# kjeffery/SimplePath

Measured on AMD Instinct MI355X. Metric: Mrays/sec (+ Msamples/sec) at fixed spp; per-pixel L2 vs CPU ref, higher is better.
Workload: dtype f32

## Files before the change

__graft_entry__.py:

```python
from __future__ import annotations

import os
import subprocess
import sys
import tempfile

ROOT = os.path.dirname(os.path.abspath(__file__))


def build() -> None:
    env = dict(os.environ)
    env.setdefault("PYTORCH_ROCM_ARCH", "gfx950")
    jobs = str(min(16, os.cpu_count() or 4))
    subprocess.run(["make", "-s", "-j", jobs, "-C", os.path.join(ROOT, "simplepath_amd")], check=True, env=env)
    subprocess.run(["make", "-s", "-C", os.path.join(ROOT, "tests", "cpp")], check=True, env=env)
    subprocess.run(["make", "-s", "-C", os.path.join(ROOT, "tests", "cpp"), "-f", "wide_visit.mk"], check=True, env=env)
    subprocess.run(["make", "-s", "-C", os.path.join(ROOT, "oracle")], check=True, env=env)
    if os.path.isdir("/root/reference") and os.path.exists(os.path.join(ROOT, "oracle", "build_ref.sh")):
        subprocess.run(["bash", os.path.join(ROOT, "oracle", "build_ref.sh")], check=True, env=env)
    if ROOT not in sys.path:
        sys.path.insert(0, ROOT)
    import simplepath_amd

    simplepath_amd.lib()


def smoke() -> None:
    if ROOT not in sys.path:
        sys.path.insert(0, ROOT)
    import numpy as np

    import simplepath_amd as sp
    from simplepath_amd import scenes
    from tests import _oracle

    d = tempfile.mkdtemp(prefix="sp_smoke_")
    scene = sp.Scene.from_file(scenes.write_bunny_scene(d))
    scene.set_resolution(64, 40)
    scene.upload(device=0, bvh_mode=1)
    tiles = np.arange(0, sp.TileScheduler(64, 40).get_num_tiles(), 3, dtype=np.int32)
    gpu, st = sp.render_tiles(scene, "direct_lighting", 2, tiles)
    cpu, _ = _oracle.render(scene, sp.string_to_integrator_type("direct_lighting"), 2, tiles, variant="spm")
    if not np.array_equal(gpu.view(np.uint32), cpu.view(np.uint32)):
        bad = int(np.sum(gpu != cpu))
        raise AssertionError(f"smoke: GPU radiance differs from the oracle in {bad} values")
    print(f"smoke ok: {tiles.size} tiles, {st.rays} rays, {st.kernel_ms:.3f} ms, bit-exact vs oracle")


if __name__ == "__main__":
    build()
    if len(sys.argv) > 1 and sys.argv[1] == "smoke":
        smoke()
```

simplepath_amd/csrc/hip/sp_mega.hpp:

```cpp
#pragma once
#include "sp_path.hpp"
#include "sp_launch.hpp"

namespace spd {
inline namespace SPD_LAYOUT_NS {

constexpr int WAVES_PER_BLOCK = 4;

template <int INTEG>
__device__ __forceinline__ rgb integrate(Ctx& c, Ray ray)
{
    if constexpr (INTEG == SP_INTEGRATOR_BRUTE_FORCE) return integrate_bruteforce(c, ray);
    else if constexpr (INTEG == SP_INTEGRATOR_BRUTE_FORCE_ITERATIVE) return integrate_iterative<false>(c, ray);
    else if constexpr (INTEG == SP_INTEGRATOR_BRUTE_FORCE_ITERATIVE_RR) return integrate_iterative<true>(c, ray);
    else if constexpr (INTEG == SP_INTEGRATOR_ITERATIVE_RRNEE) return integrate_rrnee(c, ray);
    else if constexpr (INTEG == SP_INTEGRATOR_WHITTED) return integrate_whitted(c, ray);
    else return integrate_direct(c, ray);
}


__device__ __forceinline__ Ray tail_camera_ray(const Scene& sc, uint32_t px, uint32_t py, uint32_t i, const Rsq& q)
{
    const uint32_t seed2d = ((px << 16u) | py) ^ 0x6184faf4u;
    const float    sx     = rseq_component(seed2d, sc.alpha2_0, i);
// ... 152 lines not shown
        }
    }
    asm volatile("s_waitcnt vmcnt(0)" ::: "memory");
    __builtin_amdgcn_fence(__ATOMIC_RELEASE, "agent");
    asm volatile("s_waitcnt vmcnt(0)" ::: "memory");
    if (lane == 0) __hip_atomic_store(ta.ready + k, 1u, __ATOMIC_RELAXED, __HIP_MEMORY_SCOPE_AGENT);
}

__device__ __forceinline__ void tail_chunk(const Scene& sc, const RenderArgs& args, const Rsq& q, Stack& st, int64_t j,
                                           uint32_t lane, uint32_t dx, uint32_t dy, uint32_t& rays_total,
                                           uint32_t& shadow_total, uint32_t& draws_total)
{
    const TailArgs& ta = *args.tail;
    const int64_t   k  = j / ta.chunks;
    const uint32_t  c  = (uint32_t)(j % ta.chunks);
    if (lane == 0)
        while (__hip_atomic_load(ta.ready + k, __ATOMIC_RELAXED, __HIP_MEMORY_SCOPE_AGENT) == 0u) __builtin_amdgcn_s_sleep(4);
    __builtin_amdgcn_fence(__ATOMIC_ACQUIRE, "agent");
    asm volatile("s_waitcnt vmcnt(0)" ::: "memory");
    const int64_t  slot   = args.order ? args.order[k] : k;
    const int32_t  tile   = args.tile_ids ? args.tile_ids[slot] : (int32_t)slot;
    const uint32_t px     = (uint32_t)((tile % args.tiles_x) * 8) + dx;
    const uint32_t py     = (uint32_t)((tile / args.tiles_x) * 8) + dy;
    const bool     inside = px < (uint32_t)sc.width && py < (uint32_t)sc.height;
    const size_t   p      = (size_t)k * 64 + lane;
    const uint32_t i0     = c * ta.chunk_len;
    const uint32_t i1     = min(args.spp, i0 + ta.chunk_len);
    if (!inside || i0 >= i1) return;
    const uint32_t snap = ta.snap_ctl[(size_t)c * ta.n_px + p];
    Rng            rng;
    rng.base  = ta.gens + (size_t)k * ta.gens_per_px * MT_GEN_WORDS + (size_t)lane * MT_BLK;
    rng.idx   = (int)(snap & 0xffffu);
    rng.cur   = (int)(snap >> 16);
    rng.lin   = 1;
    rng.pre   = 1;
    rng.ready = 1;
    rng.draws = 0;
    rng.pfn   = 0;
    Ctx ctx{ sc, rng, q, st, 0u, 0u };
    for (uint32_t i = i0; i < i1; ++i) {
        rng_prepare(rng);
        const float4   rec  = ta.hits[(size_t)i * ta.n_px + p];
        const uint32_t code = __float_as_uint(rec.y);
        if (code == 0xffffffffu) continue;
        const Ray   ray = tail_camera_ray(sc, px, py, i, q);
        const Hit   h{ rec.x, code, rec.z, rec.w };
        const Isect is  = finish_hit(sc, h, ray, q);
        const rgb   L   = direct_nee(ctx, is, neg(ray.d));
        ta.L[((size_t)i * 3 + 0) * ta.n_px + p] = L.r;
        ta.L[((size_t)i * 3 + 1) * ta.n_px + p] = L.g;
        ta.L[((size_t)i * 3 + 2) * ta.n_px + p] = L.b;
    }
    rays_total += ctx.rays;
    shadow_total += ctx.shadow;
    draws_total += rng.draws;
}


__device__ __forceinline__ void resume_copy_gen(const uint64_t* __restrict__ src, uint64_t* __restrict__ dst)
{
    constexpr int U = 6;
    static_assert(MT_ROWS % U == 0, "whole blocks of rows");
#pragma unroll 1
    for (int r0 = 0; r0 < MT_ROWS; r0 += U) {
        if constexpr (MT_BLK % 2 == 0) {
            ulonglong2 w[U][MT_BLK / 2];
#pragma unroll
            for (int j = 0; j < U; ++j)
#pragma unroll
                for (int b = 0; b < MT_BLK / 2; ++b)
                    w[j][b] = reinterpret_cast<const ulonglong2*>(src + (size_t)(r0 + j) * (64 * MT_BLK))[b];
#pragma unroll
            for (int j = 0; j < U; ++j)
#pragma unroll
                for (int b = 0; b < MT_BLK / 2; ++b)
                    reinterpret_cast<ulonglong2*>(dst + (size_t)(r0 + j) * (64 * MT_BLK))[b] = w[j][b];
        } else {
            uint64_t w[U][MT_BLK];
#pragma unroll
            for (int j = 0; j < U; ++j)
#pragma unroll
                for (int b = 0; b < MT_BLK; ++b) w[j][b] = src[(size_t)(r0 + j) * (64 * MT_BLK) + b];
#pragma unroll
            for (int j = 0; j < U; ++j)
#pragma unroll
                for (int b = 0; b < MT_BLK; ++b) dst[(size_t)(r0 + j) * (64 * MT_BLK) + b] = w[j][b];
        }
    }
}

__device__ __forceinline__ void resume_load(Rng& r, const ResumeArgs& ra, int64_t slot, int lane, rgb& acc)
{
    const size_t p = (size_t)slot * 64 + lane;
    resume_copy_gen(ra.gen + (size_t)slot * MT_GEN_WORDS + (size_t)lane * MT_BLK, mt_buf(r, 0));
    r.cur   = 0;
    r.idx   = (int)ra.pos[p];
    r.ready = 0;
    r.draws = 0;
    r.pfn   = 0;
#if SP_SERVE_RHO
    r.srv_on = 0;
    r.srv_A  = false;
    r.srv_B  = false;
#endif
    const float* s = ra.sum + (size_t)slot * 192 + lane;
    acc            = mkc(s[0], s[64], s[128]);
}

__device__ __forceinline__ void resume_save(Rng& r, const ResumeArgs& ra, int64_t slot, int lane, rgb acc)
{
    const size_t p  = (size_t)slot * 64 + lane;
    const bool   sw = r.idx >= MT_N && r.ready != 0;
    resume_copy_gen(mt_buf(r, sw ? mt_next(r) : r.cur), ra.gen + (size_t)slot * MT_GEN_WORDS + (size_t)lane * MT_BLK);
    ra.pos[p] = sw ? 0u : (uint32_t)r.idx;
    ra.draws[p] += r.draws;
    float* s = ra.sum + (size_t)slot * 192 + lane;
    s[0]     = acc.r;
    s[64]    = acc.g;
    s[128]   = acc.b;
}

__device__ __forceinline__ void noise_push(float& mean, float& m2, rgb L, uint32_t n)
{
    const float y = ((0.2126f * L.r) + (0.7152f * L.g)) + (0.0722f * L.b);
    if (n == 1) {
        mean = y;
        m2   = 0.0f;
    } else {
        const float d = y - mean;
        mean          = mean + d / (float)n;
        m2            = m2 + d * (y - mean);
    }
}

template <int INTEG, bool PROBE, int TAIL = 0, bool RESUME = false, bool ADAPT = false>
__device__ __forceinline__ void render_tiles_body(const Scene& sc, const RenderArgs& args, const ResumeArgs* res = nullptr,
                                                  const AdaptArgs* ad = nullptr)
{
    static_assert(!RESUME || (!PROBE && TAIL == 0), "progressive calls run the plain megakernel form");
    static_assert(!ADAPT || RESUME, "adaptive calls are progressive calls");
    extern __shared__ uint32_t lds[];
    const int tid  = threadIdx.x;
    const int lane = tid & 63;
    const int wave = tid >> 6;
    const int rs_words = rsqrt_words(sc);
    for (int i = tid; i < rs_words; i += 64 * WAVES_PER_BLOCK) lds[i] = sc.rsqrt_entries[i];
    libm_lds_init(tid, 64 * WAVES_PER_BLOCK);
#ifdef SP_WAVE_PROF
    if (lane < 16) wprof_lds[wave * 16 + lane] = 0;
#endif
#ifdef SP_TRAFFIC_DIAG
    if (lane < 32) tdg_lds[wave * 32 + lane] = 0;
#endif
    __syncthreads();
    Rsq   q{ lds };
    Stack st{ lds + rs_words + wave * sc.stack_words * 64, lane, sc.stack_depth };

    const size_t gwave = (size_t)blockIdx.x * WAVES_PER_BLOCK + wave;
    Rng          rng;
    rng.base = args.mt_state + gwave * (2 * (size_t)MT_GEN_WORDS) + (size_t)lane * MT_BLK;

    uint32_t rays_total = 0, shadow_total = 0, samples_total = 0, draws_total = 0;
    if constexpr (PROBE) rng_seed(rng, (uint32_t)(gwave * 64 + lane) ^ 0xb0ae9d99u);
    const uint32_t dx = morton_decode_1((uint32_t)lane);
    const uint32_t dy = morton_decode_1((uint32_t)lane >> 1);
    int64_t        n_active = 0;
    if constexpr (ADAPT) n_active = *ad->n_active;
    while (true) {
        int grabbed = 0;
        if (lane == 0) grabbed = atomicAdd(args.tile_counter, 1);
        const int64_t item = __shfl(grabbed, 0, 64);
        if constexpr (ADAPT) {
            if (item >= n_active) break;
        } else if constexpr (TAIL == 2) {
            {
                const int64_t NC = args.tail_cam;
                if (item < NC) {
                    fused_camera(sc, args, q, st, item, (uint32_t)lane, dx, dy);
                    continue;
                }
                const int64_t it = item - NC;
                const int64_t K = args.tail_prep, C = args.tail_items / max<int64_t>(1, K), P = min(args.tail_front, K);
                if (it >= K + args.tail_items) break;
                int64_t   idx  = it;
                bool      prep = it < P;
                if (!prep) {
                    const int64_t j = it - P, full = K - P;
                    if (j < full * (C + 1)) {
                        const int64_t g = j / (C + 1), r = j % (C + 1);
                        prep            = r == C;
                        idx             = prep ? g + P : g * C + r;
                    } else {
                        idx = full * C + (j - full * (C + 1));
                    }
                }
                if (prep) tail_prep<true>(sc, args, q, st, idx, (uint32_t)lane, dx, dy, rays_total, samples_total);
                else tail_chunk(sc, args, q, st, idx, (uint32_t)lane, dx, dy, rays_total, shadow_total, draws_total);
                continue;
            }
        } else if constexpr (TAIL == 1 || TAIL == 3) {
            if (item >= args.num_tiles + args.tail_items) break;
            if (item < args.tail_prep) {
                tail_prep<false, TAIL == 3>(sc, args, q, st, item, (uint32_t)lane, dx, dy, rays_total, samples_total);
                continue;
            }
            if (item >= args.num_tiles) {
                tail_chunk(sc, args, q, st, item - args.num_tiles, (uint32_t)lane, dx, dy, rays_total, shadow_total,
                           draws_total);
                continue;
            }
        } else if (item * (PROBE ? (int64_t)args.probe_step : 1) >= args.num_tiles) {
            break;
        }
        int64_t slot;
        if constexpr (ADAPT) slot = __builtin_amdgcn_readfirstlane(ad->active[item]);
        else slot = PROBE ? item * args.probe_step : (args.order ? args.order[item] : item);
        const uint64_t t_start = (PROBE || args.tile_diag) ? __builtin_amdgcn_s_memrealtime() : 0;
        const int32_t  tile   = args.tile_ids ? args.tile_ids[slot] : (int32_t)slot;
        const uint32_t px     = (uint32_t)((tile % args.tiles_x) * 8) + dx;
        const uint32_t py     = (uint32_t)((tile / args.tiles_x) * 8) + dy;
        const bool     inside = px < (uint32_t)sc.width && py < (uint32_t)sc.height;
        rgb            acc    = mkc(0, 0, 0);
        uint64_t       prof[4] = { 0, 0, 0, 0 };
        uint32_t       a_n0 = 0, a_more = 0;
        if constexpr (ADAPT) {
            a_n0   = __builtin_amdgcn_readfirstlane(ad->done[slot]);
            a_more = a_n0 < ad->cap ? min(ad->step, ad->cap - a_n0) : 0u;
        }
        if (inside) {
            const uint32_t pix_seed = (px << 16u) | py;
            float nz_mean = 0.0f, nz_m2 = 0.0f;
            if constexpr (ADAPT) {
                if (a_n0 == 0) {
                    rng_seed_twisted(rng, pix_seed ^ 0xb0ae9d99u);
                } else {
                    resume_load(rng, *res, slot, lane, acc);
                    nz_mean = ad->mean[(size_t)slot * 64 + lane];
                    nz_m2   = ad->m2[(size_t)slot * 64 + lane];
                }
            } else if constexpr (RESUME) {
                if (res->n0 == 0) rng_seed_twisted(rng, pix_seed ^ 0xb0ae9d99u);
                else resume_load(rng, *res, slot, lane, acc);
            } else if constexpr (!PROBE) {
                if (SP_SEED_FUSED) rng_seed_twisted(rng, pix_seed ^ 0xb0ae9d99u);
                else rng_seed(rng, pix_seed ^ 0xb0ae9d99u);
            }
            const uint32_t seed2d = pix_seed ^ 0x6184faf4u;
            Ctx c{ sc, rng, q, st, 0u, 0u };
            if (args.deep) {
                c.deep    = args.deep + gwave * 64 + lane;
                c.dstride = args.deep_stride;
            }
            uint32_t i_first = 0, i_end = args.spp;
            if constexpr (ADAPT) {
                i_first = a_n0;
                i_end   = a_n0 + a_more;
            } else if constexpr (RESUME) {
                i_first = res->n0;
                i_end   = res->n0 + args.spp;
            }
            for (uint32_t i = i_first; i < i_end; ++i) {
                rng_prepare(rng);
                const float sx = rseq_component(seed2d, sc.alpha2_0, i);
                const float sy = rseq_component(seed2d, sc.alpha2_1, i);
                const float fx = (float)(int)px + sx;
                const float fy = (float)(int)py + sy;
                Ray ray;
                ray.o = sc.camera.p;
                ray.d = normalize(add(add(scale(fx, sc.camera.vx), scale(fy, sc.camera.vy)), sc.camera.vz), q);
                if constexpr (ADAPT) {
                    rgb L;
                    if constexpr (INTEG == SP_INTEGRATOR_MANDELBROT) L = integrate_mandelbrot(fx, fy, sc.width, sc.height);
                    else SP_WPROF(0, L = integrate<INTEG>(c, ray));
                    acc = cadd(acc, L);
                    noise_push(nz_mean, nz_m2, L, i + 1u);
                } else if constexpr (INTEG == SP_INTEGRATOR_MANDELBROT)
                    acc = cadd(acc, integrate_mandelbrot(fx, fy, sc.width, sc.height));
                else
                    SP_WPROF(0, acc = cadd(acc, integrate<INTEG>(c, ray)));
            }
            if constexpr (RESUME) resume_save(rng, *res, slot, lane, acc);
            if constexpr (ADAPT) {
                ad->mean[(size_t)slot * 64 + lane] = nz_mean;
                ad->m2[(size_t)slot * 64 + lane]   = nz_m2;
            }
            acc = cdivs(acc, (float)i_end);
#ifdef SP_MEGA_PROF
            for (int k = 0; k < 4; ++k) prof[k] = c.prof[k];
#endif
            rays_total += c.rays;
            shadow_total += c.shadow;
            samples_total += ADAPT ? a_more : args.spp;
            draws_total += rng.draws;
        }
        if constexpr (ADAPT)
            if (lane == 0) ad->done[slot] = a_n0 + a_more;
        if constexpr (PROBE) {
            if (lane == 0) args.tile_time[slot] = (float)(__builtin_amdgcn_s_memrealtime() - t_start);
            continue;
        }
        if constexpr (RESUME)
            if (!args.out) continue;
        float* o = args.out + ((size_t)slot * 64 + lane) * 3;
        o[0]     = acc.r;
        o[1]     = acc.g;
        o[2]     = acc.b;
#if !defined(SP_WAVE_PROF) && !defined(SP_TRAFFIC_DIAG)
        if (args.tile_diag) {
            for (int k = 0; k < 4; ++k)
                for (int off = 32; off > 0; off >>= 1) {
                    const uint64_t o = __shfl_xor(prof[k], off, 64);
                    prof[k]          = o > prof[k] ? o : prof[k];
                }
            const uint64_t t_end  = __builtin_amdgcn_s_memrealtime();
            const uint64_t rec[8] = { t_start, t_end, (uint64_t)gwave, (uint64_t)item, prof[0], prof[1], prof[2], prof[3] };
            if (lane < 8) args.tile_diag[(size_t)slot * 8 + lane] = rec[lane];
        }
#endif
    }
#ifdef SP_WAVE_PROF
    if (args.tile_diag && lane < 16) atomicAdd(args.tile_diag + lane, wprof_lds[wave * 16 + lane]);
#endif
#ifdef SP_TRAFFIC_DIAG
    if (args.tile_diag && lane < 32) atomicAdd(args.tile_diag + 16 + lane, tdg_lds[wave * 32 + lane]);
#endif
    unsigned long long v[4] = { rays_total, shadow_total, samples_total, draws_total };
    for (int k = 0; k < 4; ++k) {
        unsigned long long s = v[k];
        for (int off = 32; off > 0; off >>= 1) s += __shfl_down(s, off, 64);
        if (lane == 0 && s) atomicAdd(args.counters + k, s);
    }
}
template <int INTEG, int MINW>
__global__ void __launch_bounds__(64 * WAVES_PER_BLOCK, MINW) sp_render_kernel(Scene sc, RenderArgs args)
{
    render_tiles_body<INTEG, false>(sc, args);
}
template <int INTEG, int MINW>
__global__ void __launch_bounds__(64 * WAVES_PER_BLOCK, MINW) sp_probe_kernel(Scene sc, RenderArgs args)
{
    render_tiles_body<INTEG, true>(sc, args);
}
template <int INTEG, int MINW>
__global__ void __launch_bounds__(64 * WAVES_PER_BLOCK, MINW) sp_resume_kernel(Scene sc, RenderArgs args, ResumeArgs res)
{
    render_tiles_body<INTEG, false, 0, true>(sc, args, &res);
}
template <int INTEG, int MINW>
__global__ void __launch_bounds__(64 * WAVES_PER_BLOCK, MINW) sp_adapt_kernel(Scene sc, RenderArgs args, ResumeArgs res, AdaptArgs ad)
{
    render_tiles_body<INTEG, false, 0, true, true>(sc, args, &res, &ad);
}
template <int MINW, bool REPLAY>
__global__ void __launch_bounds__(64 * WAVES_PER_BLOCK, MINW) sp_tail_kernel(Scene sc, RenderArgs args)
{
    render_tiles_body<SP_INTEGRATOR_DIRECT_LIGHTING, false, REPLAY ? 3 : 1>(sc, args);
}
template <int MINW>
__global__ void __launch_bounds__(64 * WAVES_PER_BLOCK, MINW) sp_fused_kernel(Scene sc, RenderArgs args)
{
    render_tiles_body<SP_INTEGRATOR_DIRECT_LIGHTING, false, 2>(sc, args);
}
}

using KernelFn = void (*)(Scene, RenderArgs);
KernelFn mega_direct(int variant);
KernelFn mega_iterative(int integ);
KernelFn mega_rrnee(int waves);
KernelFn mega_recursive(int integ);
KernelFn mega_mandelbrot();
KernelFn probe_direct(int variant);
KernelFn probe_rrnee(int waves);
KernelFn tail_direct(int variant, bool replay);
KernelFn fused_chunks();
using ResumeFn = void (*)(Scene, RenderArgs, ResumeArgs);
ResumeFn   resume_direct(int variant);
ResumeFn   resume_mandelbrot();
ResumeFn   resume_rrnee(int waves);
ResumeFn   resume_path(int integ);
ResumeFn   select_resume(int integ, int variant);
using AdaptFn = void (*)(Scene, RenderArgs, ResumeArgs, AdaptArgs);
AdaptFn    adapt_direct(int variant);
AdaptFn    adapt_mandelbrot();
AdaptFn    adapt_rrnee(int waves);
AdaptFn    adapt_path(int integ);
AdaptFn    select_adapt(int integ, int variant);

}
```

simplepath_amd/csrc/hip/sp_path.hpp:

```cpp
#pragma once
#include "sp_device.hpp"
#include "../common/sp_wide_visit.h"

namespace spd {
inline namespace SPD_LAYOUT_NS {

using namespace spm;

#ifdef SP_WAVE_PROF
static __shared__ unsigned long long wprof_lds[16 * 16];
__device__ __forceinline__ void wprof_end(int k, uint64_t t0)
{
    const uint64_t dt    = __builtin_amdgcn_s_memtime() - t0;
    const uint64_t m     = __ballot(1);
    const int      first = __ffsll((unsigned long long)m) - 1;
    if ((int)(threadIdx.x & 63) == first) {
        const int w = threadIdx.x >> 6;
        wprof_lds[w * 16 + 2 * k] += dt;
        wprof_lds[w * 16 + 2 * k + 1] += dt * (uint64_t)__popcll(m);
    }
}
#define SP_WPROF(k, stmt)                                                                                              \
    do {                                                                                                               \
        const uint64_t t_wp_ = __builtin_amdgcn_s_memtime();                                                           \
        stmt;                                                                                                          \
        wprof_end(k, t_wp_);                                                                                           \
    } while (0)
#else
#define SP_WPROF(k, stmt) stmt
#endif

#ifdef SP_TRAFFIC_DIAG
enum { TD_NODE, TD_TRI, TD_BIN, TD_HIT, TD_DRAW, TD_TOUCH, TD_SERVED, TD_TWIST, TD_SEED, TD_BOUNCE, TD_N };
static __shared__ unsigned long long tdg_lds[16 * 32];
__device__ __forceinline__ void td_add(int cat, uint64_t lines, uint64_t bytes)
{
    const uint64_t m     = __ballot(1);
    const int      first = __ffsll((unsigned long long)m) - 1;
    if ((int)(threadIdx.x & 63) == first) {
        const int w = threadIdx.x >> 6;
        tdg_lds[w * 32 + 2 * cat] += lines;
        tdg_lds[w * 32 + 2 * cat + 1] += bytes;
    }
}
__device__ __forceinline__ uint32_t td_distinct(uint64_t v, uint64_t todo)
{
    uint32_t cnt = 0;
    while (todo) {
        const int      src = __ffsll((unsigned long long)todo) - 1;
        const uint32_t lo  = (uint32_t)__shfl((int)(uint32_t)v, src, 64);
        const uint32_t hi  = (uint32_t)__shfl((int)(uint32_t)(v >> 32), src, 64);
        todo &= ~__ballot(v == (((uint64_t)hi << 32) | lo));
        ++cnt;
    }
    return cnt;
}
__device__ __forceinline__ void td_lines(int cat, const void* p, int nbytes)
{
    const uint64_t a = (uint64_t)(uintptr_t)p, l0 = a >> 7, l1 = (a + (uint64_t)nbytes - 1) >> 7;
    const uint64_t m = __ballot(1);
    uint32_t cnt = td_distinct(l0, m);
    cnt += td_distinct(l1 != l0 ? l1 : ~0ull, __ballot(l1 != l0));
    td_add(cat, cnt, (uint64_t)__popcll(m) * (uint64_t)nbytes);
}
__device__ __forceinline__ void td_twist(int cat)
{
    const uint64_t m = __ballot(1);
    uint64_t groups = 0;
    for (int g = 0; g < 16; ++g) groups += ((m >> (4 * g)) & 0xfull) ? 1 : 0;
    td_add(cat, groups * 78 * 2, (uint64_t)__popcll(m) * 312 * 8 * 2);
}
#define SP_TD(stmt) stmt
#else
#define SP_TD(stmt)
#endif

struct Rsq {
    const uint32_t* t;
};
__device__ __forceinline__ float rsqrt_ref(float a, const Rsq& q)
{
    const uint4    h  = *reinterpret_cast<const uint4*>(q.t);
    const uint32_t hi = q.t[4];
    RsqrtTable     tb{ q.t + RSQ_HDR, (int32_t)h.x, h.y, h.z, (int32_t)h.w, hi };
    return rsqrt_newton(a, rsqrtss_emulated(a, tb));
}
__device__ __forceinline__ f3 normalize(f3 a, const Rsq& q) { return scale(a, rsqrt_ref(dot(a, a), q)); }

#ifndef SP_SQRT_UNIT
#define SP_SQRT_UNIT 1
#endif
__device__ __forceinline__ float sqrt_unit(float x)
{
#if SP_SQRT_UNIT
    const float s  = __builtin_amdgcn_sqrtf(x);
    const float sd = __uint_as_float(__float_as_uint(s) - 1u);
    const float su = __uint_as_float(__float_as_uint(s) + 1u);
    const float vp = __builtin_fmaf(-sd, s, x);
    const float vs = __builtin_fmaf(-su, s, x);
    float       r  = (vp <= 0.0f) ? sd : s;
    r              = (vs > 0.0f) ? su : r;
    return r;
#else
    return sqrt_f(x);
#endif
}

#ifndef SP_RNG_PF
#define SP_RNG_PF 2
#endif
#ifndef SP_XP_SERVED_FREE
#define SP_XP_SERVED_FREE 0
#endif
constexpr int RNG_PF = SP_RNG_PF;
struct Rng {
    uint64_t* base;
    int       cur;
    int       idx;
    int       ready;
    uint32_t  draws;
    int       lin = 0, pre = 0;
    int       pfn = 0;
#ifdef SP_TRAFFIC_DIAG
    int       td_cat = TD_DRAW;
#endif
    uint64_t  pf[RNG_PF > 0 ? RNG_PF : 1];
#if SP_SERVE_RHO
    int       srv_on  = 0;
    bool      srv_A = false, srv_B = false;
    uint32_t  srv_pos = 0, srv_dc = 0, srv_coat = 0, srv_posA = 0, srv_pwA = 0;
#endif
};

__device__ __forceinline__ uint64_t* mt_buf(Rng& r, int b) { return r.base + (size_t)b * MT_GEN_WORDS; }
__device__ __forceinline__ int       mt_next(const Rng& r) { return r.lin ? r.cur + 1 : r.cur ^ 1; }

#ifndef SP_TWIST_BLOCK
#define SP_TWIST_BLOCK 12
#endif
#ifndef SP_TWIST_SKIP_BLOCK
#define SP_TWIST_SKIP_BLOCK 12
#endif
template <int NW, bool SECOND>
__device__ __forceinline__ void mt_twist_words(const uint64_t* __restrict__ A, uint64_t* __restrict__ B, int k, uint64_t& ak)
{
    if constexpr (NW > 0) {
        uint64_t a1[NW], am[NW];
#pragma unroll
        for (int j = 0; j < NW; ++j) {
            a1[j] = A[mt_off(k + j + 1)];
            am[j] = SECOND ? B[mt_off(k + j - (MT_N - MT_M))] : A[mt_off(k + j + MT_M)];
        }
#pragma unroll
        for (int j = 0; j < NW; ++j) {
            B[mt_off(k + j)] = am[j] ^ mt_mix(ak, a1[j]);
// ... 1795 lines not shown
        rho_accumulate(r, mf_sample_geom(m, p, wo, u2, u1, q), m.microfacet_r, grey);
    }
    if (grey) r.g = r.b = r.r;
    return cdivs(r, (float)16u);
}

#if SP_SERVE_RHO
#ifndef SP_MERGE_QUERIES
#define SP_MERGE_QUERIES 1
#endif
enum : int {
    MQ_O = 0,
    MQ_D3 = 192,
    MQ_T3 = 384,
    MQ_D1 = 448,
    MQ_T1 = 640,
    MQ_BEST = 704,
    MQ_ANY = 832,
    MQ_TB = 896,
    MQ_Q = 960,
    MQ_CNT = 992,
    MQ_WORDS = 996,
    SRV_W = 0, SRV_REQ = 512, SRV_WORDS = 576,
    SRV_WAVE_WORDS = (SP_MERGE_QUERIES && MQ_WORDS > SRV_WORDS) ? MQ_WORDS : SRV_WORDS
};
static_assert(SRV_WAVE_WORDS % 4 == 0 && MQ_BEST % 2 == 0, "u64 LDS atomics need 8-byte alignment");
struct MqLayout {
    enum : int { O = MQ_O, D3 = MQ_D3, T3 = MQ_T3, D1 = MQ_D1, T1 = MQ_T1, BEST = MQ_BEST, AMAX = MQ_BEST, ANY = MQ_ANY,
                 TB = MQ_TB, Q = MQ_Q, CNT = MQ_CNT };
};
#ifndef SP_MQ_SHADOW
#define SP_MQ_SHADOW 1
#endif
static __shared__ __attribute__((aligned(16))) uint32_t srv_lds[4][SRV_WAVE_WORDS];
__device__ __forceinline__ float*   srv_w_at(int wave, int k, int j) { return reinterpret_cast<float*>(&srv_lds[wave][SRV_W + (k * 2 + j) * 64]); }
__device__ __forceinline__ uint8_t* srv_req_of(int wave) { return reinterpret_cast<uint8_t*>(&srv_lds[wave][SRV_REQ]); }
#endif

template <bool PAIR = (SP_RNG_PAIR != 0), bool ALIGN = (SP_RHO_ALIGNED != 0), bool TOUCH = (SP_RHO_TOUCH != 0)>
__device__ __forceinline__ void glossy_weights(const Material& m, f3 wo, Rng& rng, const Rsq& q, float w[2])
{
#if SP_SERVE_RHO
    if (rng.srv_on == 1) {
        const uint32_t d = rng.draws - rng.srv_pos;
        int            k = -1;
        if (rng.srv_A && rng.draws == rng.srv_posA) k = 3;
        else if (rng.srv_B) k = (d == 0u) ? 0 : (d == rng.srv_dc) ? 1 : (d == 2u * rng.srv_dc + rng.srv_coat) ? 2 : -1;
        if (k >= 0) {
            const int lane = threadIdx.x & 63, wave = threadIdx.x >> 6;
            w[0]           = srv_w_at(wave, k, 0)[lane];
            w[1]           = srv_w_at(wave, k, 1)[lane];
            rng_skip_reserved(rng, (int)rng.srv_dc);
            return;
        }
    }
#endif
    rgb r0;
    SP_WPROF(1, r0 = (mf_rho16<PAIR, ALIGN, TOUCH>(m, wo, rng, q)));
    const rgb r1 = cscale(m.lambert_albedo, k_pi);
    float     sum = 0.0f;
    w[0] = luminance(r0);
    sum += w[0];
    w[1] = luminance(r1);
    sum += w[1];
    w[0] = w[0] / sum;
    w[1] = w[1] / sum;
}
__device__ __forceinline__ float lambert_only_weight(const Material& m)
{
    const rgb r   = cscale(m.lambert_albedo, k_pi);
    float     sum = 0.0f;
    float     w   = luminance(r);
    sum += w;
    return w / sum;
}
__device__ __forceinline__ float balance(float p, float inner) { return (inner == 0.0f) ? 0.0f : p / inner; }

__device__ __forceinline__ MSample lambert_sample(const Material& m, Rng& rng)
{
    MSample r;
    const P2 u = next2D(rng);
    r.dir      = sample_uniform_hemisphere(u);
    r.color    = m.lambert_albedo;
    r.pdf      = k_uniform_hemisphere_pdf;
    r.props    = PROP_DIFFUSE | PROP_REFLECTIVE;
    return r;
}

__device__ __forceinline__ MSample onesample_sample_w(const Material& m, f3 wo, const float w[2], Rng& rng, const Rsq& q)
{
    const float u   = next1D(rng);
    float       cdf = 0.0f;
    int         sel = 1;
    for (int i = 0; i < 2; ++i) {
        if (w[i] + cdf > u) { sel = i; break; }
        cdf += w[i];
    }
    MSample res = (sel == 0) ? mf_sample(m, wo, rng, q) : lambert_sample(m, rng);
    if (res.pdf == 0.0f || cblack(res.color)) {
        MSample z;
        z.color = mkc(0, 0, 0); z.dir = mk(0, 0, 0); z.pdf = 0.0f; z.props = 0;
        return z;
    }
    const f3 wi = res.dir;
    rgb      values[2];
    float    pdfs[2];
    for (int i = 0; i < 2; ++i) {
        if (i == sel) {
            values[i] = res.color;
            pdfs[i]   = res.pdf * w[i];
        } else if (i == 0) {
            values[i] = mf_eval(m, wo, wi, q);
            pdfs[i]   = mf_pdf(m, wo, wi, q) * w[i];
        } else {
            values[i] = m.lambert_albedo;
            pdfs[i]   = k_uniform_hemisphere_pdf * w[i];
        }
    }
    const float inner = (0.0f + pdfs[0]) + pdfs[1];
    rgb         col   = mkc(0, 0, 0);
    float       pdf   = 0.0f;
    for (int i = 0; i < 2; ++i) {
        if (pdfs[i] > 0.0f) {
            const float mw = balance(pdfs[i], inner);
            col            = cadd(col, cscale(values[i], mw));
            pdf += pdfs[i];
        }
    }
    MSample out;
    out.color = col;
    out.dir   = wi;
    out.pdf   = pdf;
    out.props = res.props;
    return out;
}
__device__ __forceinline__ MSample onesample_sample(const Material& m, f3 wo, Rng& rng, const Rsq& q)
{
    if (m.kind == SP_MAT_LAMBERTIAN) return lambert_sample(m, rng);
    float w[2];
    glossy_weights(m, wo, rng, q, w);
    return onesample_sample_w(m, wo, w, rng, q);
}

__device__ __forceinline__ rgb onesample_eval_w(const Material& m, f3 wo, f3 wi, const float w[2], const Rsq& q)
{
    const float p0    = mf_pdf(m, wo, wi, q) * w[0];
    const float p1    = k_uniform_hemisphere_pdf * w[1];
    const float inner = (0.0f + p0) + p1;
    rgb         r     = mkc(0, 0, 0);
    if (p0 > 0.0f) r = cadd(r, cscale(mf_eval(m, wo, wi, q), balance(p0, inner)));
    if (p1 > 0.0f) r = cadd(r, cscale(m.lambert_albedo, balance(p1, inner)));
    return r;
}
__device__ __forceinline__ rgb onesample_eval(const Material& m, f3 wo, f3 wi, Rng& rng, const Rsq& q)
{
    if (m.kind == SP_MAT_LAMBERTIAN) {
        const float w     = lambert_only_weight(m);
        const float p     = k_uniform_hemisphere_pdf * w;
        const float inner = 0.0f + p;
        rgb         r     = mkc(0, 0, 0);
        if (p > 0.0f) r = cadd(r, cscale(m.lambert_albedo, balance(p, inner)));
        return r;
    }
    float w[2];
    glossy_weights(m, wo, rng, q, w);
    return onesample_eval_w(m, wo, wi, w, q);
}

__device__ __forceinline__ float onesample_pdf_w(const Material& m, f3 wo, f3 wi, const float w[2], const Rsq& q)
{
    float p = 0.0f;
    p += w[0] * mf_pdf(m, wo, wi, q);
    p += w[1] * k_uniform_hemisphere_pdf;
    return p;
}
__device__ __forceinline__ float onesample_pdf(const Material& m, f3 wo, f3 wi, Rng& rng, const Rsq& q)
{
    if (m.kind == SP_MAT_LAMBERTIAN) {
        const float w = lambert_only_weight(m);
        float       p = 0.0f;
        p += w * k_uniform_hemisphere_pdf;
        return p;
    }
    float w[2];
    glossy_weights(m, wo, rng, q, w);
    return onesample_pdf_w(m, wo, wi, w, q);
}

__device__ __forceinline__ bool material_has_rho(const Scene& sc, int mid)
{
    const Material& m = sc.materials[mid];
    const int       k = (m.kind == SP_MAT_CLEARCOAT) ? sc.materials[m.base].kind : m.kind;
    return k == SP_MAT_GLOSSY;
}

__device__ __forceinline__ MSample material_sample_local(const Scene& sc, int mid, f3 wo, Rng& rng, const Rsq& q)
{
    const Material& m    = sc.materials[mid];
    const bool      coat = m.kind == SP_MAT_CLEARCOAT;
    float           f    = 0.0f;
    if (coat) {
        f             = fresnel_dielectric(wo.y, 1.0f, m.coat_ior);
        const float u = next1D(rng);
        if (u < f) {
            MSample s;
            s.dir   = mk(-wo.x, wo.y, -wo.z);
            s.color = cdivs(cscale(m.coat_color, f), abs_f(s.dir.y));
            s.pdf   = f;
            s.props = PROP_SPECULAR | PROP_REFLECTIVE;
            return s;
        }
    }
    const MSample b = onesample_sample(sc.materials[coat ? m.base : mid], wo, rng, q);
    if (!coat || b.pdf == 0.0f) return b;
    MSample s;
    s.pdf   = (1.0f - f) * b.pdf;
    s.color = cmul(csub(mkc(1, 1, 1), cscale(m.coat_color, f)), b.color);
    s.dir   = b.dir;
    s.props = b.props;
    return s;
}
__device__ __forceinline__ rgb material_eval_local(const Scene& sc, int mid, f3 wo, f3 wi, Rng& rng, const Rsq& q)
{
    const Material& m    = sc.materials[mid];
    const bool      coat = m.kind == SP_MAT_CLEARCOAT;
    const rgb       r    = onesample_eval(sc.materials[coat ? m.base : mid], wo, wi, rng, q);
    if (!coat) return r;
    const float f = fresnel_dielectric(wo.y, 1.0f, m.coat_ior);
    return cscale(r, 1.0f - f);
}
__device__ __forceinline__ float material_pdf_local(const Scene& sc, int mid, f3 wo, f3 wi, Rng& rng, const Rsq& q)
{
    const Material& m    = sc.materials[mid];
    const bool      coat = m.kind == SP_MAT_CLEARCOAT;
    const float     p    = onesample_pdf(sc.materials[coat ? m.base : mid], wo, wi, rng, q);
    if (!coat) return p;
    const float f = fresnel_dielectric(wo.y, 1.0f, m.coat_ior);
    return (1.0f - f) * p;
}

__device__ __forceinline__ MSample material_sample(const Scene& sc, int mid, f3 wo_w, f3 n, Rng& rng, const Rsq& q)
{
    const Onb o = onb_from_v(n, q);
    MSample   r = material_sample_local(sc, mid, to_onb(o, wo_w), rng, q);
    if (r.pdf == 0.0f || cblack(r.color)) return r;
    r.dir = to_world(o, r.dir);
    return r;
}
__device__ __forceinline__ rgb material_eval(const Scene& sc, int mid, f3 wo, f3 wi, f3 n, Rng& rng, const Rsq& q)
{
    const Onb o = onb_from_v(n, q);
    return material_eval_local(sc, mid, to_onb(o, wo), to_onb(o, wi), rng, q);
}
__device__ __forceinline__ float material_pdf(const Scene& sc, int mid, f3 wo, f3 wi, f3 n, Rng& rng, const Rsq& q)
{
    const Onb o = onb_from_v(n, q);
    return material_pdf_local(sc, mid, to_onb(o, wo), to_onb(o, wi), rng, q);
}

struct LSample {
    rgb   L;
    float pdf;
    Ray   ray;
    float tmin, tmax;
};

__device__ __forceinline__ float sphere_pdf(const Light& l, f3 observer_world)
{
    const f3    obs = xfm_point(l.w2o, observer_world);
    const float sqr = dot(obs, obs);
    if (sqr <= 1.0f) return k_uniform_sphere_pdf;
    constexpr float sin2_1_5_deg = 0.00068523f;
    const float     sin2_max     = 1.0f / sqr;
    const float     cos_max      = sqrt_unit(std_max(0.0f, 1.0f - sin2_max));
    const float     omc          = (sin2_max < sin2_1_5_deg) ? sin2_max / 2.0f : 1.0f - cos_max;
    return 1.0f / (2.0f * k_pi * omc);
}

__device__ __forceinline__ LSample light_sample(const Scene& sc, const Light& l, f3 obs, f3 obs_n, P2 u, const Rsq& q)
{
    LSample s;
    f3      wi;
    float   pdf, max_dist;
    s.L = l.radiance;
    if (l.kind == SP_LIGHT_SPHERE) {
        const f3 lo = xfm_point(l.w2o, obs);
        f3       local;
        if (dot(lo, lo) <= 1.0f) {
            local = sample_uniform_sphere(u);
        } else {
            const f3  smp = sample_cosine_hemisphere(u);
            const Onb o   = onb_from_v(lo, q);
            local         = to_world(o, smp);
        }
        const f3 sp_w = xfm_point(l.o2w, local);
        const f3 sn_w = xfm_vector(l.nrm, local);
        const f3 to_sample = sub(sp_w, obs);
        wi                 = normalize(to_sample, q);
        pdf                = sphere_pdf(l, obs);
        max_dist           = length(to_sample) - ray_offset(sn_w, neg(wi));
    } else if (l.kind == SP_LIGHT_IMAGE_ENVIRONMENT) {
        const EnvSample es = env_sample(sc.envs[l.image], u);
        wi                 = es.wi;
        pdf                = es.pdf;
        s.L                = es.L;
        max_dist           = k_infinite;
    } else {
        wi       = sample_uniform_sphere(u);
        pdf      = k_uniform_sphere_pdf;
        max_dist = k_infinite;
    }
    s.pdf   = pdf;
    s.tmin  = ray_offset(obs_n, wi);
    s.tmax  = max_dist;
    s.ray.o = obs;
    s.ray.d = wi;
    return s;
}
__device__ __forceinline__ float light_pdf(const Scene& sc, const Light& l, f3 obs, f3 wi)
{
    if (l.kind == SP_LIGHT_SPHERE) return sphere_pdf(l, obs);
    if (l.kind == SP_LIGHT_IMAGE_ENVIRONMENT) return env_pdf(sc.envs[l.image], wi);
    return k_uniform_sphere_pdf;
}

#ifndef SP_OCC_CACHE
#define SP_OCC_CACHE 0
#endif
struct Ctx {
    const Scene& sc;
    Rng&         rng;
    const Rsq&   q;
    Stack        st;
    uint32_t     rays, shadow;
    uint32_t     occ_slot = 0xffffffffu;
    float*       deep    = nullptr;
    size_t       dstride = 0;
#ifdef SP_MEGA_PROF
    uint64_t prof[4] = { 0, 0, 0, 0 };
#endif
};
#ifdef SP_MEGA_PROF
#define SP_PROF(k, stmt)                                                                                               \
    do {                                                                                                               \
        const uint64_t t_prof_ = __builtin_amdgcn_s_memtime();                                                         \
        stmt;                                                                                                          \
        c.prof[k] += __builtin_amdgcn_s_memtime() - t_prof_;                                                           \
    } while (0)
#else
#define SP_PROF(k, stmt) stmt
#endif

__device__ __forceinline__ bool occluded(Ctx& c, const Ray& r, float tmin, float tmax)
{
    ++c.shadow;
    ++c.rays;
    bool hit;
    SP_WPROF(3, hit = scene_any(c.sc, r, tmin, tmax, c.st, SP_OCC_CACHE ? &c.occ_slot : nullptr));
    return hit;
}

struct Query {
    LightHit lh;
    bool     geom;
    Isect    is;
};
__device__ __forceinline__ Query trace(Ctx& c, const Ray& ray, float tmin, float tmax)
{
    Query qr;
    ++c.rays;
    Hit h;
    SP_WPROF(2, {
        qr.lh = scene_intersect_lights(c.sc, ray, tmin, tmax, c.st);
        if (qr.lh.hit) tmax = qr.lh.t;
        h = scene_intersect(c.sc, ray, tmin, tmax, c.st);
    });
    qr.geom     = (h.code != 0xffffffffu);
    if (qr.geom) qr.is = finish_hit(c.sc, h, ray, c.q);
    return qr;
}

__device__ __forceinline__ rgb direct_nee(Ctx& c, const Isect& is, f3 wo)
{
    rgb L = mkc(0, 0, 0);
    for (int li = 0; li < c.sc.n_lights; ++li) {
        const Light l = uload_light(c.sc.lights + li);
        LSample     ls;
        SP_PROF(1, ls = light_sample(c.sc, l, is.p, is.n, next2D(c.rng), c.q));
        if (ls.pdf == 0.0f || cblack(ls.L)) continue;
        const f3 wi = ls.ray.d;
        rgb      f;
        SP_PROF(2, f = material_eval(c.sc, is.material, wo, wi, is.n, c.rng, c.q));
        bool vis = false;
        if (!cblack(f)) SP_PROF(3, vis = !occluded(c, ls.ray, ls.tmin, ls.tmax));
        if (vis) L = cadd(L, cdivs(cscale(cmul(f, ls.L), abs_f(dot(wi, is.n))), ls.pdf));
    }
    return L;
}

__device__ __forceinline__ uint32_t sample_draws(const Scene& sc, const Isect& is, f3 wo, const Rsq& q)
{
    const Material& m    = sc.materials[is.material];
    const int       base = (m.kind == SP_MAT_CLEARCOAT) ? sc.materials[m.base].kind : m.kind;
    bool            rho  = false;
    if (base != SP_MAT_LAMBERTIAN) {
        const Onb o = onb_from_v(is.n, q);
        rho         = to_onb(o, wo).y != 0.0f;
    }
    uint32_t n = 0;
    for (int li = 0; li < sc.n_lights; ++li) {
        const Light lt  = uload_light(sc.lights + li);
        const float pdf = (lt.kind == SP_LIGHT_SPHERE) ? sphere_pdf(lt, is.p) : k_uniform_sphere_pdf;
        n += 2;
        if (rho && !(pdf == 0.0f || cblack(lt.radiance))) n += 32;
    }
    return n;
}

__device__ __forceinline__ rgb integrate_direct(Ctx& c, Ray ray)
{
    rgb L = mkc(0, 0, 0);
    if (0 >= c.sc.max_depth) return L;
    Query qr;
    SP_PROF(0, qr = trace(c, ray, k_ray_epsilon, k_infinite));
    if (qr.geom) {
        L = direct_nee(c, qr.is, neg(ray.d));
    } else if (qr.lh.hit) {
        L = cadd(L, cmul(mkc(1, 1, 1), light_hit_L(c.sc, qr.lh, ray.d, c.q)));
    }
    return L;
}

template <bool RR>
__device__ __forceinline__ rgb integrate_iterative(Ctx& c, Ray ray)
{
    rgb   throughput = mkc(1, 1, 1);
    rgb   L          = mkc(0, 0, 0);
    float tmin = k_ray_epsilon, tmax = k_infinite;
    constexpr float rr_cut = 0.1f;
    for (int depth = 0; depth < c.sc.max_depth; ++depth) {
        rng_prepare(c.rng);
        const Query qr = trace(c, ray, tmin, tmax);
        if (qr.geom) {
            const f3      wo = neg(ray.d);
            const f3      n  = qr.is.n;
            const MSample s  = material_sample(c.sc, qr.is.material, wo, n, c.rng, c.q);
            if (s.pdf == 0.0f || cblack(s.color)) break;
            const f3    wi     = s.dir;
            const float cosine = abs_f(dot(wi, n));
            throughput         = cmul(throughput, cdivs(cscale(s.color, cosine), s.pdf));
            if (RR && depth >= c.sc.rr_depth) {
                const float lum = luminance(throughput);
                if (lum < rr_cut) {
                    const float qv = std_max(0.05f, lum / rr_cut);
                    if (next1D(c.rng) < qv) throughput = cdivs(throughput, qv);
                    else break;
                }
            }
            ray.o = ray_at(ray, qr.is.t);
            ray.d = wi;
            tmin  = ray_offset(cosine);
            tmax  = k_infinite;
        } else if (qr.lh.hit) {
            L = cadd(L, cmul(throughput, light_hit_L(c.sc, qr.lh, ray.d, c.q)));
            break;
        } else {
            break;
        }
    }
    return L;
}

constexpr int MAX_RECURSION = 32;
__device__ __forceinline__ rgb integrate_bruteforce(Ctx& c, Ray ray)
{
    float cosv[MAX_RECURSION];
    rgb   colv[MAX_RECURSION];
    float pdfv[MAX_RECURSION];
    int   depth = 0;
    rgb   Lend  = mkc(0, 0, 0);
    const bool deep = c.deep != nullptr;
    const int  maxd = deep ? c.sc.max_depth : (c.sc.max_depth < MAX_RECURSION ? c.sc.max_depth : MAX_RECURSION);
    auto put = [&](int k, float cs, rgb col, float pdf) {
        if (!deep) { cosv[k] = cs; colv[k] = col; pdfv[k] = pdf; return; }
        float* d = c.deep + (size_t)k * 5 * c.dstride;
        d[0] = cs; d[c.dstride] = col.r; d[2 * c.dstride] = col.g; d[3 * c.dstride] = col.b; d[4 * c.dstride] = pdf;
    };
    while (true) {
        if (depth >= maxd) { Lend = mkc(0, 0, 0); break; }
        rng_prepare(c.rng);
        const Query qr = trace(c, ray, k_ray_epsilon, k_infinite);
        if (qr.geom) {
            const f3      wo = neg(ray.d);
            const f3      n  = qr.is.n;
            const MSample s  = material_sample(c.sc, qr.is.material, wo, n, c.rng, c.q);
            if (s.pdf == 0.0f || cblack(s.color)) { Lend = mkc(0, 0, 0); break; }
            put(depth, dot(s.dir, n), s.color, s.pdf);
            ray.o       = ray_at(ray, qr.is.t);
            ray.d       = s.dir;
            ++depth;
        } else if (qr.lh.hit) {
            Lend = light_hit_L(c.sc, qr.lh, ray.d, c.q);
            break;
        } else {
            Lend = mkc(0, 0, 0);
            break;
        }
    }
    for (int k = depth - 1; k >= 0; --k) {
        float cs, pdf;
        rgb   col;
        if (!deep) { cs = cosv[k]; col = colv[k]; pdf = pdfv[k]; }
        else {
            const float* d = c.deep + (size_t)k * 5 * c.dstride;
            cs = d[0]; col = mkc(d[c.dstride], d[2 * c.dstride], d[3 * c.dstride]); pdf = d[4 * c.dstride];
        }
        Lend = cdivs(cmul(cscale(Lend, cs), col), pdf);
    }
    return Lend;
}

__device__ __forceinline__ rgb integrate_whitted(Ctx& c, Ray ray)
{
    rgb        Lv[MAX_RECURSION + 1];
    int        depth = 0;
    const bool deep  = c.deep != nullptr;
    const int  maxd  = deep ? c.sc.max_depth : (c.sc.max_depth < MAX_RECURSION ? c.sc.max_depth : MAX_RECURSION);
    auto put = [&](int k, rgb L) {
        if (!deep) { Lv[k] = L; return; }
        float* d = c.deep + (size_t)k * 3 * c.dstride;
        d[0] = L.r; d[c.dstride] = L.g; d[2 * c.dstride] = L.b;
    };
    auto get = [&](int k) {
        if (!deep) return Lv[k];
        const float* d = c.deep + (size_t)k * 3 * c.dstride;
        return mkc(d[0], d[c.dstride], d[2 * c.dstride]);
    };
    while (true) {
        rgb L = mkc(0, 0, 0);
        if (depth >= maxd) { put(depth, L); break; }
        rng_prepare(c.rng);
        const Query qr   = trace(c, ray, k_ray_epsilon, k_infinite);
        bool        more = false;
        if (qr.geom) {
            const f3 wo = neg(ray.d);
            L           = direct_nee(c, qr.is, wo);
            if (depth < c.sc.max_depth) {
                const MSample s = material_sample(c.sc, qr.is.material, wo, qr.is.n, c.rng, c.q);
// ... 501 lines not shown
```

Before: 4023.

## Reorder NEE to trace shadow ray first and skip glossy weights when occluded

Direct-light NEE now casts the shadow ray before evaluating glossy material weights. When the ray is occluded and interval bounds prove whether the contribution is black, the costly glossy_weights RNG-driven estimate is skipped and its 32 RNG draws are reserved and skipped to keep the sequence aligned. This removes per-light BRDF estimation on occluded samples. The trade-off is shadow rays are now traced even when the BRDF would have been black, and the ray/shadow counters are adjusted to match the old accounting. A debug check mode is added behind a macro.

```diff
diff --git a/__graft_entry__.py b/__graft_entry__.py
--- a/__graft_entry__.py
+++ b/__graft_entry__.py
@@ -15,6 +15,7 @@
     subprocess.run(["make", "-s", "-j", jobs, "-C", os.path.join(ROOT, "simplepath_amd")], check=True, env=env)
     subprocess.run(["make", "-s", "-C", os.path.join(ROOT, "tests", "cpp")], check=True, env=env)
     subprocess.run(["make", "-s", "-C", os.path.join(ROOT, "tests", "cpp"), "-f", "wide_visit.mk"], check=True, env=env)
+    subprocess.run(["make", "-s", "-j", "3", "-C", os.path.join(ROOT, "tests", "cpp"), "-f", "nee_order.mk"], check=True, env=env)
     subprocess.run(["make", "-s", "-C", os.path.join(ROOT, "oracle")], check=True, env=env)
     if os.path.isdir("/root/reference") and os.path.exists(os.path.join(ROOT, "oracle", "build_ref.sh")):
         subprocess.run(["bash", os.path.join(ROOT, "oracle", "build_ref.sh")], check=True, env=env)
diff --git a/simplepath_amd/csrc/common/sp_nee_black.h b/simplepath_amd/csrc/common/sp_nee_black.h
--- /dev/null
+++ b/simplepath_amd/csrc/common/sp_nee_black.h
@@ -0,0 +1,76 @@
+#pragma once
+
+#include "sp_math.h"
+
+namespace spn {
+using namespace spm;
+
+enum : int { NEE_UNKNOWN = 0, NEE_BLACK = 1, NEE_NOT_BLACK = 2 };
+
+constexpr float k_hemi_pdf = 1.0f / (2.0f * k_pi);
+
+constexpr float k_wo_y_min   = 0x1p-10f;
+constexpr float k_wo_len_lo  = 0.998f, k_wo_len_hi = 1.002f;
+constexpr float k_alpha_min  = 0x1p-6f, k_alpha_max = 2.0f;
+constexpr float k_ior_min    = 1.0f, k_ior_max = 8.0f;
+constexpr float k_r_max      = 16.0f;
+constexpr float k_est_max    = 0x1p32f;
+constexpr float k_pe_max     = 0x1p30f;
+constexpr float k_albedo_max = 0x1p10f, k_albedo_top_min = 0x1p-12f;
+constexpr float k_lum_min    = 0x1p-10f, k_lum_max = 0x1p10f;
+constexpr float k_coat_min   = 0x1p-30f, k_coat_max = 2.0f;
+
+SP_HD float balance(float p, float inner) { return (inner == 0.0f) ? 0.0f : p / inner; }
+
+SP_HD float lambert_lum(rgb albedo) { return luminance(cscale(albedo, k_pi)); }
+
+SP_HD void weights_from(float r0, float A, float w[2])
+{
+    float sum = 0.0f;
+    w[0] = r0;
+    sum += w[0];
+    w[1] = A;
+    sum += w[1];
+    w[0] = w[0] / sum;
+    w[1] = w[1] / sum;
+}
+
+SP_HD rgb nee_finish(float P, rgb E, rgb albedo, const float w[2], bool coat, float cf)
+{
+    const float p0    = P * w[0];
+    const float p1    = k_hemi_pdf * w[1];
+    const float inner = (0.0f + p0) + p1;
+    rgb         r     = mkc(0, 0, 0);
+    if (p0 > 0.0f) r = cadd(r, cscale(E, balance(p0, inner)));
+    if (p1 > 0.0f) r = cadd(r, cscale(albedo, balance(p1, inner)));
+    return coat ? cscale(r, cf) : r;
+}
+
+SP_HD bool estimate_bounded(f3 wo, float alpha_x, float alpha_y, float ior, rgb R, bool visible_area)
+{
+    const float l2 = dot(wo, wo);
+    bool        ok = visible_area;
+    ok = ok && abs_f(wo.y) >= k_wo_y_min && l2 >= k_wo_len_lo && l2 <= k_wo_len_hi;
+    ok = ok && alpha_x >= k_alpha_min && alpha_x <= k_alpha_max && alpha_y >= k_alpha_min && alpha_y <= k_alpha_max;
+    ok = ok && ior >= k_ior_min && ior <= k_ior_max;
+    ok = ok && R.r >= 0.0f && R.r <= k_r_max && R.g >= 0.0f && R.g <= k_r_max && R.b >= 0.0f && R.b <= k_r_max;
+    return ok;
+}
+
+SP_HD int nee_black_known(bool bounded, float P, rgb E, rgb albedo, float A, bool coat, float cf)
+{
+    bool ok = bounded;
+    ok = ok && P >= 0.0f && P <= k_pe_max;
+    ok = ok && E.r >= 0.0f && E.r <= k_pe_max && E.g >= 0.0f && E.g <= k_pe_max && E.b >= 0.0f && E.b <= k_pe_max;
+    ok = ok && albedo.r >= 0.0f && albedo.r <= k_albedo_max && albedo.g >= 0.0f && albedo.g <= k_albedo_max &&
+         albedo.b >= 0.0f && albedo.b <= k_albedo_max;
+    ok = ok && (albedo.r >= k_albedo_top_min || albedo.g >= k_albedo_top_min || albedo.b >= k_albedo_top_min);
+    ok = ok && A >= k_lum_min && A <= k_lum_max;
+    if (!ok) return NEE_UNKNOWN;
+    if (!coat) return NEE_NOT_BLACK;
+    if (cf == 0.0f) return NEE_BLACK;
+    const float a = abs_f(cf);
+    return (a >= k_coat_min && a <= k_coat_max) ? NEE_NOT_BLACK : NEE_UNKNOWN;
+}
+
+}
diff --git a/simplepath_amd/csrc/hip/sp_mega.hpp b/simplepath_amd/csrc/hip/sp_mega.hpp
--- a/simplepath_amd/csrc/hip/sp_mega.hpp
+++ b/simplepath_amd/csrc/hip/sp_mega.hpp
@@ -328,6 +328,9 @@
 #ifdef SP_TRAFFIC_DIAG
     if (lane < 32) tdg_lds[wave * 32 + lane] = 0;
 #endif
+#if SP_XP_NEE_CHECK
+    if (lane < 16) nee_chk_lds[wave * 16 + lane] = 0;
+#endif
     __syncthreads();
     Rsq   q{ lds };
     Stack st{ lds + rs_words + wave * sc.stack_words * 64, lane, sc.stack_depth };
@@ -481,7 +484,7 @@
         o[0]     = acc.r;
         o[1]     = acc.g;
         o[2]     = acc.b;
-#if !defined(SP_WAVE_PROF) && !defined(SP_TRAFFIC_DIAG)
+#if !defined(SP_WAVE_PROF) && !defined(SP_TRAFFIC_DIAG) && !SP_XP_NEE_CHECK
         if (args.tile_diag) {
             for (int k = 0; k < 4; ++k)
                 for (int off = 32; off > 0; off >>= 1) {
@@ -496,6 +499,12 @@
     }
 #ifdef SP_WAVE_PROF
     if (args.tile_diag && lane < 16) atomicAdd(args.tile_diag + lane, wprof_lds[wave * 16 + lane]);
+#endif
+#if SP_XP_NEE_CHECK
+    if (args.tile_diag && lane < 16) {
+        if (lane == 10) atomicMax(args.tile_diag + lane, nee_chk_lds[wave * 16 + lane]);
+        else atomicAdd(args.tile_diag + lane, nee_chk_lds[wave * 16 + lane]);
+    }
 #endif
 #ifdef SP_TRAFFIC_DIAG
     if (args.tile_diag && lane < 32) atomicAdd(args.tile_diag + 16 + lane, tdg_lds[wave * 32 + lane]);
diff --git a/simplepath_amd/csrc/hip/sp_path.hpp b/simplepath_amd/csrc/hip/sp_path.hpp
--- a/simplepath_amd/csrc/hip/sp_path.hpp
+++ b/simplepath_amd/csrc/hip/sp_path.hpp
@@ -1,6 +1,7 @@
 #pragma once
 #include "sp_device.hpp"
 #include "../common/sp_wide_visit.h"
+#include "../common/sp_nee_black.h"
 
 namespace spd {
 inline namespace SPD_LAYOUT_NS {
@@ -2102,16 +2103,18 @@
     if (p1 > 0.0f) r = cadd(r, cscale(m.lambert_albedo, balance(p1, inner)));
     return r;
 }
+__device__ __forceinline__ rgb lambert_eval(const Material& m)
+{
+    const float w     = lambert_only_weight(m);
+    const float p     = k_uniform_hemisphere_pdf * w;
+    const float inner = 0.0f + p;
+    rgb         r     = mkc(0, 0, 0);
+    if (p > 0.0f) r = cadd(r, cscale(m.lambert_albedo, balance(p, inner)));
+    return r;
+}
 __device__ __forceinline__ rgb onesample_eval(const Material& m, f3 wo, f3 wi, Rng& rng, const Rsq& q)
 {
-    if (m.kind == SP_MAT_LAMBERTIAN) {
-        const float w     = lambert_only_weight(m);
-        const float p     = k_uniform_hemisphere_pdf * w;
-        const float inner = 0.0f + p;
-        rgb         r     = mkc(0, 0, 0);
-        if (p > 0.0f) r = cadd(r, cscale(m.lambert_albedo, balance(p, inner)));
-        return r;
-    }
+    if (m.kind == SP_MAT_LAMBERTIAN) return lambert_eval(m);
     float w[2];
     glossy_weights(m, wo, rng, q, w);
     return onesample_eval_w(m, wo, wi, w, q);
@@ -2310,6 +2313,13 @@
     return hit;
 }
 
+__device__ __forceinline__ bool shadow_walk(Ctx& c, const Ray& r, float tmin, float tmax)
+{
+    bool hit;
+    SP_WPROF(3, hit = scene_any(c.sc, r, tmin, tmax, c.st, SP_OCC_CACHE ? &c.occ_slot : nullptr));
+    return hit;
+}
+
 struct Query {
     LightHit lh;
     bool     geom;
@@ -2330,20 +2340,93 @@
     return qr;
 }
 
+#ifndef SP_XP_NEE_CHECK
+#define SP_XP_NEE_CHECK 0
+#endif
+#if SP_XP_NEE_CHECK
+static __shared__ unsigned long long nee_chk_lds[16 * 16];
+__device__ __forceinline__ void nee_count(int k, unsigned long long n = 1ull) { atomicAdd(&nee_chk_lds[(threadIdx.x >> 6) * 16 + k], n); }
+__device__ __forceinline__ void nee_check(Ctx& c, const Material& mb, f3 wol, float P, rgb E, float A, bool coat, float cf, int known,
+                                          bool occ, bool run)
+{
+    const uint64_t vote  = __builtin_amdgcn_ballot_w64(true);
+    const bool     first = (threadIdx.x & 63) == __builtin_ctzll(vote);
+    const bool     vis   = __builtin_amdgcn_ballot_w64(!occ) != 0ull;
+    if (first) nee_count(run ? 1 : 0);
+    if (first && run && !vis) nee_count(2);
+    if (run && occ && known != spn::NEE_UNKNOWN) nee_count(3);
+    if (occ && known == spn::NEE_UNKNOWN) nee_count(4);
+    nee_count(5);
+    Rng   rc = c.rng;
+    float w[2];
+    glossy_weights(mb, wol, rc, c.q, w);
+    const bool black = cblack(spn::nee_finish(P, E, mb.lambert_albedo, w, coat, cf));
+    if (known != spn::NEE_UNKNOWN && black != (known == spn::NEE_BLACK)) nee_count(6);
+    if (!(w[0] >= 0.0f && w[0] <= 1.0f && w[1] >= 0.0f && w[1] <= 1.0f)) nee_count(7);
+    if (!run) nee_count(8);
+    if (!run && known == spn::NEE_BLACK) nee_count(9);
+    if (w[0] >= 0.0f) atomicMax(&nee_chk_lds[(threadIdx.x >> 6) * 16 + 10], (unsigned long long)f2u(w[0]));
+}
+#endif
+#ifndef SP_NEE_SKIP
+#define SP_NEE_SKIP 2
+#endif
 __device__ __forceinline__ rgb direct_nee(Ctx& c, const Isect& is, f3 wo)
 {
-    rgb L = mkc(0, 0, 0);
+    rgb             L    = mkc(0, 0, 0);
+    const Material& m    = c.sc.materials[is.material];
+    const bool      coat = m.kind == SP_MAT_CLEARCOAT;
+    const Material& mb   = c.sc.materials[coat ? m.base : is.material];
+    const bool      rho  = mb.kind != SP_MAT_LAMBERTIAN;
     for (int li = 0; li < c.sc.n_lights; ++li) {
         const Light l = uload_light(c.sc.lights + li);
         LSample     ls;
         SP_PROF(1, ls = light_sample(c.sc, l, is.p, is.n, next2D(c.rng), c.q));
         if (ls.pdf == 0.0f || cblack(ls.L)) continue;
-        const f3 wi = ls.ray.d;
-        rgb      f;
-        SP_PROF(2, f = material_eval(c.sc, is.material, wo, wi, is.n, c.rng, c.q));
-        bool vis = false;
-        if (!cblack(f)) SP_PROF(3, vis = !occluded(c, ls.ray, ls.tmin, ls.tmax));
-        if (vis) L = cadd(L, cdivs(cscale(cmul(f, ls.L), abs_f(dot(wi, is.n))), ls.pdf));
+        const f3    wi  = ls.ray.d;
+        const Onb   o   = onb_from_v(is.n, c.q);
+        const f3    wol = to_onb(o, wo), wil = to_onb(o, wi);
+        const float cf  = coat ? 1.0f - fresnel_dielectric(wol.y, 1.0f, m.coat_ior) : 1.0f;
+        rgb         f   = mkc(0, 0, 0);
+        if (!rho) {
+            f = lambert_eval(mb);
+            if (coat) f = cscale(f, cf);
+        }
+        const bool walk = rho || !cblack(f);
+        bool       occ  = false;
+        if (walk) SP_PROF(3, occ = shadow_walk(c, ls.ray, ls.tmin, ls.tmax));
+        bool black = !walk;
+        if (rho) {
+            const float P     = mf_pdf(mb, wol, wil, c.q);
+            const rgb   E     = mf_eval(mb, wol, wil, c.q);
+            const float A     = spn::lambert_lum(mb.lambert_albedo);
+            const int   known = spn::nee_black_known(
+                spn::estimate_bounded(wol, mb.alpha_x, mb.alpha_y, mb.microfacet_ior, mb.microfacet_r, mb.sample_visible_area != 0),
+                P, E, mb.lambert_albedo, A, coat, cf);
+            const bool mine = !occ || known == spn::NEE_UNKNOWN;
+            bool       run  = mine || SP_NEE_SKIP == 0;
+#if SP_NEE_SKIP == 1
+            const bool some = __builtin_amdgcn_ballot_w64(mine) != 0ull;
+            run             = run || some;
+#endif
+#if SP_XP_NEE_CHECK
+            nee_check(c, mb, wol, P, E, A, coat, cf, known, occ, run);
+#endif
+            if (run) {
+                float w[2];
+                SP_PROF(2, glossy_weights(mb, wol, c.rng, c.q, w));
+                f     = spn::nee_finish(P, E, mb.lambert_albedo, w, coat, cf);
+                black = cblack(f);
+            } else {
+                rng_reserve(c.rng, 32);
+                rng_skip_reserved(c.rng, 32);
+                black = known == spn::NEE_BLACK;
+            }
+        }
+        if (black) continue;
+        ++c.shadow;
+        ++c.rays;
+        if (!occ) L = cadd(L, cdivs(cscale(cmul(f, ls.L), abs_f(dot(wi, is.n))), ls.pdf));
     }
     return L;
 }
```

Measured after the change: 4230, median of 6. 1.05x the previous value.
